# oritwoen/vgen

Hardware: AMD Instinct MI355X
Metric: Mkeys/sec (keys tried per second) (higher is better)
Workload: dtype u32

## Files before the change

vgen_amd/csrc/device/kernels.hip:

```cpp
#include <hip/hip_runtime.h>

#ifndef VG_PARK
#define VG_PARK 0
#endif
#ifndef VG_KECCAK_BLOCK
#define VG_KECCAK_BLOCK 1
#endif
#ifndef VG_PARKI
#define VG_PARKI 1
#endif
#define VG_HASH_BLOCKS 1
#include "../core/dfa_eval.h"
#include "../core/ec.h"
#include "../core/ed25519.h"
#include "../core/filter_eval.h"
#include "../core/hash.h"
#include "../core/rnd.h"
#include "../core/taproot.h"
#include "device_types.h"
#include "launch.h"

namespace vg {

constexpr int WG = SEQ_WG;

#ifndef VG_SEQ_WAVES_P2TR
#define VG_SEQ_WAVES_P2TR 2
#endif
#ifndef VG_SEQ_WAVES_ETH
#define VG_SEQ_WAVES_ETH 4
#endif


__device__ __forceinline__ void lds_store_fe(u32 *base, int stride, int col, const fe &a) {
#pragma unroll
    for (int i = 0; i < 9; i++) base[i * stride + col] = a.n[i];
}

__device__ __forceinline__ void lds_load_fe(const u32 *base, int stride, int col, fe &a) {
#pragma unroll
    for (int i = 0; i < 9; i++) a.n[i] = base[i * stride + col];
}

typedef __attribute__((address_space(3))) volatile u32 lds_vu32;

__device__ __forceinline__ void lds_park_fe(u32 *base, int stride, int col, const fe &a) {
    lds_vu32 *b = (lds_vu32 *)base;
#pragma unroll
    for (int i = 0; i < 9; i++) b[i * stride + col] = a.n[i];
}

__device__ __forceinline__ void lds_unpark_fe(u32 *base, int stride, int col, fe &a) {
    lds_vu32 *b = (lds_vu32 *)base;
#pragma unroll
    for (int i = 0; i < 9; i++) a.n[i] = b[i * stride + col];
}

__device__ __forceinline__ void fe_set_beta(fe &b) {
    b.n[0] = 0x119501EEu; b.n[1] = 0x09CB6143u; b.n[2] = 0x1D626570u; b.n[3] = 0x0092EA25u; b.n[4] = 0x034E99CFu;
    b.n[5] = 0x03CF561Au; b.n[6] = 0x1C41B991u; b.n[7] = 0x056CAF80u; b.n[8] = 0x007AE96Au;
}

__device__ __forceinline__ void shfl_xor_fe(fe &r, const fe &a, int mask) {
#pragma unroll
    for (int i = 0; i < 9; i++) r.n[i] = (u32)__shfl_xor((int)a.n[i], mask);
}

__device__ __forceinline__ u32 match_slot(DevMatchHeader *hdr, bool hit, u32 match_base) {
    const unsigned long long m = __ballot(hit);
    if (m == 0) return 0xFFFFFFFFu;
    const u32 rank = __builtin_amdgcn_mbcnt_hi((u32)(m >> 32), __builtin_amdgcn_mbcnt_lo((u32)m, 0u));
    const int leader = __ffsll((long long)m) - 1;
    u32 first = 0;
    if (hit && rank == 0) first = atomicAdd(&hdr->count, (u32)__popcll(m));
    first = (u32)__builtin_amdgcn_readlane((int)first, leader);
    return first + rank - match_base;
}

#include "hash_blocks.inc"


template <int FMT>
struct MatchFmt {
    static constexpr int value = (FMT == VGF_P2TR || vgf_is_eth(FMT)) ? -1 : FMT;
};

template <int FMT>
struct DumpOnly {
    static constexpr bool value = FMT == VGF_ETHEREUM_CONTRACT;
};

template <int FMT>
struct PayloadWords {
    static constexpr int value = (FMT == VGF_P2TR) ? 8 : 5;
};

template <int FMT, bool LONE = false>
__device__ __forceinline__ bool payload_from_point(const fe &x, const fe &y_canon, u32 *out) {
    static_assert(FMT != VGF_P2TR, "taproot payloads come from p2tr_tweak_kernel / p2tr_out_kernel");
    static_assert(!LONE || FMT == VGF_P2PKH, "the lone variant exists for the headline format only");
    u32 xw[8];
    fe_to_words(x, xw);
    if (LONE) {
        u32 sha[8];
        sha256_pub33(2u | (y_canon.n[0] & 1u), xw, sha);
        ripemd160_of_sha(sha, out);
    } else if (FMT == VGF_P2PKH || FMT == VGF_P2WPKH) {
        hash160_pub33_block(2u | (y_canon.n[0] & 1u), xw, out);
    } else if (FMT == VGF_P2SH_P2WPKH) {
        u32 h[5];
        hash160_pub33_block(2u | (y_canon.n[0] & 1u), xw, h);
        hash160_script22_block(h, out);
    } else if (FMT == VGF_P2PKH_UNCOMPRESSED) {
        u32 yw[8];
        fe_to_words(y_canon, yw);
        hash160_pub65_block(xw, yw, out);
    } else {
        u32 yw[8];
        fe_to_words(y_canon, yw);
#if VG_KECCAK_BLOCK
        keccak_addr_block(xw, yw, out);
#else
        keccak256_pub64_addr(xw, yw, out);
#endif
        if (FMT == VGF_ETHEREUM_CONTRACT) {
            u32 acc[5];
#pragma unroll
            for (int i = 0; i < 5; i++) acc[i] = out[i];
#if VG_KECCAK_BLOCK
            keccak_create_block(acc, out);
#else
            keccak256_create_addr(acc, out);
#endif
        }
    }
    return true;
}



__global__ void __launch_bounds__(WG) __attribute__((amdgpu_waves_per_eu(1, 8)))
seq_fwd_kernel(const SeqArgs args) {
    __builtin_amdgcn_s_setprio(3);
    __shared__ u32 tree[9 * WG];
    const int tid = threadIdx.x;
    const u32 S = args.s;
    const u32 lanes = args.lanes;
    const u32 u = blockIdx.x * WG + tid;

    fe rx;
#pragma unroll
    for (int i = 0; i < 9; i++) rx.n[i] = args.rtab[(size_t)i * lanes + u];

    u32 *pre = args.pre + u;
    fe acc;
#pragma unroll 1
    for (u32 j = 0; j < S; j++) {
        fe dx;
#pragma unroll
        for (int i = 0; i < 9; i++) dx.n[i] = rx.n[i] + args.q[j].nqx[i];
        if (j == 0) {
            acc = dx;
            fe_normalize_weak(acc);
        } else {
            fe_mul(acc, acc, dx);
        }
#pragma unroll
        for (int i = 0; i < 9; i++) pre[(size_t)(j * 9 + i) * lanes] = acc.n[i];
    }

    fe sib, pair;
    shfl_xor_fe(sib, acc, 1);
    fe_mul(pair, acc, sib);
    if ((tid & 1) == 0) lds_store_fe(tree, WG, WG / 2 + (tid >> 1), pair);
    __syncthreads();
    for (int width = WG / 4; width >= 1; width >>= 1) {
        if (tid < width) {
            const int k = width + tid;
            fe a, b, p;
            lds_load_fe(tree, WG, 2 * k, a);
            lds_load_fe(tree, WG, 2 * k + 1, b);
            fe_mul(p, a, b);
            lds_store_fe(tree, WG, k, p);
        }
        __syncthreads();
    }
    u32 *tg = args.tree + (size_t)blockIdx.x * 9 * WG;
#pragma unroll
    for (int i = 0; i < 9; i++) tg[i * WG + tid] = tree[i * WG + tid];
    if (tid < 9) args.root[(size_t)tid * args.groups + blockIdx.x] = tree[tid * WG + 1];
}


__global__ void __launch_bounds__(64) seq_inv_kernel(u32 *root, u32 groups) {
    __builtin_amdgcn_s_setprio(3);
    const u32 g = blockIdx.x * 64 + threadIdx.x;
    const u32 gg = g < groups ? g : groups - 1;
    fe r, ri;
#pragma unroll
    for (int i = 0; i < 9; i++) r.n[i] = root[(size_t)i * groups + gg];
    fe_inv(ri, r);
    if (g < groups) {
#pragma unroll
        for (int i = 0; i < 9; i++) root[(size_t)i * groups + g] = ri.n[i];
    }
}


__device__ __forceinline__ void tree_down_sweep(u32 *tree, int tid) {
    static_assert(WG % 64 == 0 && WG >= 128, "siblings c and c ^ 1 must be lanes of one 64-lane wave at every level");
    for (int width = 1; width <= WG / 4; width <<= 1) {
        if (tid < 2 * width) {
            const int c = 2 * width + tid;
            fe ik, sib, ic;
            lds_load_fe(tree, WG, c >> 1, ik);
            lds_load_fe(tree, WG, c ^ 1, sib);
            fe_mul(ic, ik, sib);
            __builtin_amdgcn_wave_barrier();
            lds_store_fe(tree, WG, c, ic);
        }
        __syncthreads();
    }
}

#ifndef VG_SEQ_WAVES_P2PKH
#define VG_SEQ_WAVES_P2PKH 4
#endif
#ifndef VG_SEQ_WAVES_P2SH
#define VG_SEQ_WAVES_P2SH 4
#endif
#ifndef VG_SEQ_WAVES_UNCOMP
#define VG_SEQ_WAVES_UNCOMP 4
#endif
#ifndef VG_SEQ_WAVES_FULL20
#define VG_SEQ_WAVES_FULL20 4
#endif
#ifndef VG_SEQ_WAVES_EC
#define VG_SEQ_WAVES_EC 4
#endif
#ifndef VG_SEQ_WAVES_HASH
#define VG_SEQ_WAVES_HASH 8
#endif
#ifndef VG_BASE_PRIO
#define VG_BASE_PRIO 1
#endif
#ifndef VG_EC_PRIO
#define VG_EC_PRIO 0
#endif
#ifndef VG_EC_SPRIO
#define VG_EC_SPRIO 0
#endif
#ifndef VG_SEQ_WAVES_HASH_FULL
#define VG_SEQ_WAVES_HASH_FULL 6
#endif
template <int FMT, bool FULL, bool ENDO = false>
struct SeqWaves {
    static constexpr int value = FMT == VGF_P2TR ? VG_SEQ_WAVES_P2TR : vgf_is_eth(FMT) ? (FULL && ENDO ? 3 : VG_SEQ_WAVES_ETH)
                                 : FULL ? VG_SEQ_WAVES_FULL20 : FMT == VGF_P2SH_P2WPKH ? VG_SEQ_WAVES_P2SH
                                 : FMT == VGF_P2PKH_UNCOMPRESSED ? VG_SEQ_WAVES_UNCOMP : VG_SEQ_WAVES_P2PKH;
};

template <int FMT, bool FULL, bool ENDO = false, bool LONE = false, bool SPLIT = false>
__global__ void __launch_bounds__(WG) __attribute__((amdgpu_waves_per_eu(SPLIT ? VG_SEQ_WAVES_EC : SeqWaves<FMT, FULL, ENDO>::value, SPLIT ? VG_SEQ_WAVES_EC : SeqWaves<FMT, FULL, ENDO>::value)))
seq_bwd_kernel(const SeqArgs args) {
#if VG_BASE_PRIO
    if (!SPLIT) __builtin_amdgcn_s_setprio(VG_BASE_PRIO);
#endif
#if VG_EC_PRIO
    if (SPLIT) __builtin_amdgcn_s_setprio(VG_EC_PRIO);
#endif
    static_assert(!SPLIT || (!FULL && !ENDO && !LONE && FMT == VGF_P2PKH), "the split form parks compressed keys: x and the parity of y");
    __shared__ u32 tree[9 * WG];
    __shared__ u32 ypark[ENDO && (FMT == VGF_P2PKH_UNCOMPRESSED || vgf_is_eth(FMT)) ? 9 * WG : 1];
    extern __shared__ u32 dyn_lds[];
    constexpr int NW = PayloadWords<FMT>::value;
    constexpr int PARKM = (!FULL && !ENDO && !LONE && (FMT == VGF_P2PKH || FMT == VGF_P2WPKH)) ? VG_PARK : 0;
    constexpr bool PARK = PARKM == 1, PARK2 = PARKM == 2;
    constexpr bool PARKI = VG_PARKI && !PARK && !PARK2 && !LONE && (FMT == VGF_P2PKH_UNCOMPRESSED || vgf_is_eth(FMT) || (FMT == VGF_P2PKH && FULL && ENDO));
    __shared__ u32 rpark[PARK ? 17 * WG : (PARK2 || PARKI) ? 9 * WG : 1];
    constexpr bool LEANMUL = !(FULL && ENDO) && (FMT == VGF_P2PKH || FMT == VGF_P2WPKH || FMT == VGF_P2SH_P2WPKH);
    const int tid = threadIdx.x;
    const GenTables gtab{args.gtab, args.gtab16, args.gtab_bits};
    u32 *dfa_lds = dyn_lds;
    if (FULL) {
        for (u32 i = tid; i < args.dfa_bytes / 4; i += WG) dfa_lds[i] = args.dfa_blob[i];
    }
    const u32 S = args.s;
    const u32 lanes = args.lanes;
    const u32 u = blockIdx.x * WG + tid;
    const bool stamp = FMT != VGF_P2TR && !SPLIT && blockIdx.x == 0 && args.mhdr != nullptr;
    const unsigned long long stamp_c0 = stamp ? clock64() : 0ull, stamp_w0 = stamp ? wall_clock64() : 0ull;

    const u32 *tg = args.tree + (size_t)blockIdx.x * 9 * WG;
#pragma unroll
    for (int i = 0; i < 9; i++) tree[i * WG + tid] = tg[i * WG + tid];
    __syncthreads();
    if (tid < 9) tree[tid * WG + 1] = args.root[(size_t)tid * args.groups + blockIdx.x];
    __syncthreads();
    tree_down_sweep(tree, tid);
    const u32 *pre = args.pre + u;
    fe inv;
    {
        fe ip, sib;
        lds_load_fe(tree, WG, WG / 2 + (tid >> 1), ip);
#pragma unroll
        for (int i = 0; i < 9; i++) sib.n[i] = args.pre[(size_t)((S - 1) * 9 + i) * lanes + (u ^ 1u)];
        fe_mul(inv, ip, sib);
    }
    if (ENDO || PARK || PARK2) __syncthreads();

    fe rx, ry;
    if (!PARK2) {
#pragma unroll
        for (int i = 0; i < 9; i++) {
            rx.n[i] = args.rtab[(size_t)i * lanes + u];
            ry.n[i] = args.rtab[(size_t)(9 + i) * lanes + u];
        }
    }
    if (PARK2) lds_park_fe(tree, WG, tid, inv);
    if (PARKI) lds_park_fe(rpark, WG, tid, inv);
    if (PARK) {
        lds_park_fe(rpark, WG, tid, rx);
        {
            lds_vu32 *b = (lds_vu32 *)(rpark + 9 * WG);
#pragma unroll
            for (int i = 0; i < 8; i++) b[i * WG + tid] = ry.n[i];
        }
        lds_park_fe(tree, WG, tid, inv);
    }

    const u32 half = args.n >> 1;
    const bool dump = DumpOnly<FMT>::value || args.dump != nullptr;
    fe zrun;
    u32 step = 0;

#pragma unroll 1
    for (int j = (int)S - 1; j >= 0; j--) {
        const DevSeqQ &q = args.q[j];
        fe dx, idx;
        if (PARK) {
            lds_unpark_fe(rpark, WG, tid, rx);
            lds_unpark_fe(tree, WG, tid, inv);
        }
        if (PARKI) lds_unpark_fe(rpark, WG, tid, inv);
        if (PARK2) {
            const u32 *rt = args.rtab + u;
            asm volatile("" : "+v"(rt));
#pragma unroll
            for (int i = 0; i < 9; i++) rx.n[i] = rt[(size_t)i * lanes];
            lds_unpark_fe(tree, WG, tid, inv);
        }
#pragma unroll
        for (int i = 0; i < 9; i++) dx.n[i] = rx.n[i] + q.nqx[i];
        if (j > 0) {
            fe pj;
#pragma unroll
            for (int i = 0; i < 9; i++) pj.n[i] = pre[(size_t)((j - 1) * 9 + i) * lanes];
            fe_mul(idx, inv, pj);
            fe_mul(inv, inv, dx);
            if (PARK || PARK2) lds_park_fe(tree, WG, tid, inv);
            if (PARKI) lds_park_fe(rpark, WG, tid, inv);
        } else {
            idx = inv;
        }
        if (PARK2) lds_park_fe(rpark, WG, tid, idx);
        if (!PARK && !PARK2) {
#pragma unroll
            for (int i = 0; i < 9; i++) {
                asm volatile("" : "+v"(rx.n[i]));
                asm volatile("" : "+v"(ry.n[i]));
            }
        }
        fe nsum, nqy;
        if (!PARK2) fe_neg(nsum, rx, 1);
#pragma unroll
        for (int i = 0; i < 9; i++) {
            if (!PARK2) nsum.n[i] += q.nqx[i];
            nqy.n[i] = q.nqy[i];
        }
#pragma unroll 1
        for (int sgn = 0; sgn < 2; sgn++) {
            fe dy, lam, x3, t, y3;
            if (PARK2) {
                const u32 *rt = args.rtab + u;
                asm volatile("" : "+v"(rt));
#pragma unroll
                for (int i = 0; i < 9; i++) {
                    rx.n[i] = rt[(size_t)i * lanes];
                    ry.n[i] = rt[(size_t)(9 + i) * lanes];
                }
                fe_neg(nsum, rx, 1);
#pragma unroll
                for (int i = 0; i < 9; i++) nsum.n[i] += q.nqx[i];
                lds_unpark_fe(rpark, WG, tid, idx);
            }
            if (PARK) {
                lds_vu32 *b = (lds_vu32 *)(rpark + 9 * WG);
#pragma unroll
                for (int i = 0; i < 8; i++) ry.n[i] = b[i * WG + tid];
            }
            if (sgn) fe_neg(dy, ry, 1);
            else dy = ry;
#pragma unroll
            for (int i = 0; i < 9; i++) dy.n[i] += q.nqy[i];
            fe_mul(lam, dy, idx);
            fe_sqr_add<LEANMUL>(x3, lam, nsum);
            if (VG_EC_SPRIO && !LONE) __builtin_amdgcn_s_setprio(0);
            fe_canonicalize_product(x3);
            fe_neg(t, x3, 1);
#pragma unroll
            for (int i = 0; i < 9; i++) t.n[i] += q.qx[i];
            if (VG_EC_SPRIO && !LONE) __builtin_amdgcn_s_setprio(VG_BASE_PRIO);
            fe_mul_add<LEANMUL>(y3, lam, t, nqy);
            if (VG_EC_SPRIO && !LONE) __builtin_amdgcn_s_setprio(0);
            if (FMT == VGF_P2PKH || FMT == VGF_P2WPKH || FMT == VGF_P2SH_P2WPKH)
                y3.n[0] = fe_parity_weak(y3);
            else
                fe_canonicalize_product(y3);

            if (FMT == VGF_P2TR) {
                gej qq;
                const bool okq = taproot_tweak_point(x3, y3, gtab, qq);
                const bool zero = taproot_z_is_zero(qq.z);
                if (zero) fe_set_one(qq.z);
                if (step == 0) zrun = qq.z;
                else fe_mul(zrun, zrun, qq.z);
                u32 *o = args.tq + (size_t)step * 27 * lanes + u;
#pragma unroll
                for (int i = 0; i < 9; i++) {
                    o[(size_t)i * lanes] = qq.x.n[i];
                    o[(size_t)(9 + i) * lanes] = qq.z.n[i];
                    o[(size_t)(18 + i) * lanes] = zrun.n[i];
                }
                args.tq_flag[(size_t)step * lanes + u] = (okq && !zero) ? 1u : 0u;
                step++;
                continue;
            }

            if (SPLIT) {
                u32 xw[8];
                fe_to_words(x3, xw);
                u32 *o = args.xs + (size_t)((u32)j * 2u + (u32)sgn) * lanes + u;
#pragma unroll
                for (int i = 0; i < 8; i++) o[(size_t)i * args.n] = xw[i];
                o[(size_t)8 * args.n] = 2u | (y3.n[0] & 1u);
                continue;
            }
            const u32 index = sgn ? (half - (u + 1) * S + (u32)j) : (half + u * S + (u32)j);
            if (ENDO) {
                constexpr bool NEEDS_Y = FMT == VGF_P2PKH_UNCOMPRESSED || vgf_is_eth(FMT);
                const u32 ypar = y3.n[0] & 1u;
                lds_park_fe(tree, WG, tid, x3);
                if (NEEDS_Y) lds_park_fe(ypark, WG, tid, y3);
#pragma unroll 1
                for (u32 v = 0; v < 6; v++) {
                    const u32 e = v >> 1, sneg = v & 1u;
                    fe xe, ye;
                    lds_unpark_fe(tree, WG, tid, xe);
                    if (sneg == 0 && e > 0) {
                        fe beta;
                        fe_set_beta(beta);
                        fe_mul(xe, xe, beta);
                        fe_canonicalize_product(xe);
                        lds_park_fe(tree, WG, tid, xe);
                    }
                    if (NEEDS_Y) {
                        lds_unpark_fe(ypark, WG, tid, ye);
                        if (sneg) {
                            fe ny;
                            fe_neg(ny, ye, 1);
                            fe_normalize(ny);
                            ye = ny;
                        }
                    } else {
                        ye.n[0] = ypar ^ sneg;
                    }
                    u32 ple[NW];
                    (void)payload_from_point<FMT == VGF_P2TR ? VGF_P2PKH : FMT>(xe, ye, ple);
                    const u32 vindex = (sneg * 3u + e) * args.n + index;
                    if (dump) {
                        u32 *o = args.dump + (size_t)vindex * NW;
#pragma unroll
                        for (int i = 0; i < NW; i++) o[i] = ple[i];
                    } else {
                        const bool hit = FULL ? dfa_match_payload_n<NW, MatchFmt<FMT>::value>(dfa_lds, (int)args.fmt, ple) : filter_eval_n<NW>(args.filter, ple);
                        const u32 slot = match_slot(args.mhdr, hit, args.match_base);
                        if (hit && slot < args.match_cap) {
                            DevMatch *m = args.mrec + slot;
                            m->index = vindex;
                            m->reserved = 0;
#pragma unroll
                            for (int i = 0; i < 8; i++) m->payload[i] = i < NW ? ple[i] : 0u;
                        }
                    }
                }
                continue;
            }

            u32 pl[NW];
            const bool ok = payload_from_point<FMT == VGF_P2TR ? VGF_P2PKH : FMT, LONE>(x3, y3, pl);

            if (dump) {
                u32 *o = args.dump + (size_t)index * NW;
#pragma unroll
                for (int i = 0; i < NW; i++) o[i] = ok ? pl[i] : 0u;
            } else {
                const bool hit = ok && (FULL ? dfa_match_payload_n<NW, MatchFmt<FMT>::value>(dfa_lds, (int)args.fmt, pl) : filter_eval_n<NW>(args.filter, pl));
                const u32 slot = match_slot(args.mhdr, hit, args.match_base);
                if (hit && slot < args.match_cap) {
                    DevMatch *m = args.mrec + slot;
                    m->index = index;
                    m->reserved = 0;
#pragma unroll
                    for (int i = 0; i < 8; i++) m->payload[i] = i < NW ? pl[i] : 0u;
                }
            }
        }
    }
    if (stamp && tid == 0) {
        args.mhdr->clk_cycles += (u32)(clock64() - stamp_c0);
        args.mhdr->clk_ticks += (u32)(wall_clock64() - stamp_w0);
    }
    if (FMT == VGF_P2TR) {
        __syncthreads();
        fe sib, pair;
        shfl_xor_fe(sib, zrun, 1);
        fe_mul(pair, zrun, sib);
        if ((tid & 1) == 0) lds_store_fe(tree, WG, WG / 2 + (tid >> 1), pair);
        __syncthreads();
#pragma unroll 1
        for (int width = WG / 4; width >= 1; width >>= 1) {
            if (tid < width) {
                const int k = width + tid;
                fe a, b, p;
                lds_load_fe(tree, WG, 2 * k, a);
                lds_load_fe(tree, WG, 2 * k + 1, b);
                fe_mul(p, a, b);
                lds_store_fe(tree, WG, k, p);
            }
            __syncthreads();
        }
        u32 *t2 = args.tree2 + (size_t)blockIdx.x * 9 * WG;
#pragma unroll
        for (int i = 0; i < 9; i++) t2[i * WG + tid] = tree[i * WG + tid];
        if (tid < 9) args.root2[(size_t)tid * args.groups + blockIdx.x] = tree[tid * WG + 1];
    }
}

template <int FMT, bool FULL>
struct HashWaves {
    static constexpr int value = FULL && FMT == VGF_P2PKH ? VG_SEQ_WAVES_HASH_FULL : VG_SEQ_WAVES_HASH;
};
template <int FMT, bool FULL>
__global__ void __launch_bounds__(WG) __attribute__((amdgpu_waves_per_eu(HashWaves<FMT, FULL>::value, HashWaves<FMT, FULL>::value)))
seq_hash_kernel(const SeqArgs args) {
#if VG_BASE_PRIO
    __builtin_amdgcn_s_setprio(VG_BASE_PRIO);
#endif
    static_assert(FMT == VGF_P2PKH || FMT == VGF_P2SH_P2WPKH, "compressed-key formats (P2WPKH shares P2PKH's payload)");
    extern __shared__ u32 dfa_lds[];
    const int tid = threadIdx.x;
    if (FULL) {
        for (u32 i = tid; i < args.dfa_bytes / 4; i += WG) dfa_lds[i] = args.dfa_blob[i];
        __syncthreads();
    }
    const u32 lanes = args.lanes, S = args.s, half = args.n >> 1;
    const u32 u = blockIdx.x * WG + tid;
    const bool stamp = blockIdx.x == 0 && blockIdx.y == 0 && args.mhdr != nullptr;
    const unsigned long long stamp_c0 = stamp ? clock64() : 0ull, stamp_w0 = stamp ? wall_clock64() : 0ull;
    const bool dump = args.dump != nullptr;
#pragma unroll 1
    for (u32 k = 0; k < args.hash_kpl; k++) {
        const u32 step = blockIdx.y * args.hash_kpl + k;
        const u32 *in = args.xs + (size_t)step * lanes + u;
        u32 xw[8];
#pragma unroll
        for (int i = 0; i < 8; i++) xw[i] = in[(size_t)i * args.n];
        const u32 prefix = in[(size_t)8 * args.n];
        u32 pl[5];
        if (FMT == VGF_P2SH_P2WPKH) {
            u32 h[5];
            hash160_pub33_block(prefix, xw, h);
            hash160_script22_block(h, pl);
        } else {
            hash160_pub33_block(prefix, xw, pl);
        }
        const u32 j = step >> 1, sgn = step & 1u;
        const u32 index = sgn ? (half - (u + 1) * S + j) : (half + u * S + j);
        if (dump) {
            u32 *o = args.dump + (size_t)index * 5;
#pragma unroll
            for (int i = 0; i < 5; i++) o[i] = pl[i];
        } else {
            const bool hit = FULL ? dfa_match_payload_n<5, MatchFmt<FMT>::value>(dfa_lds, (int)args.fmt, pl) : filter_eval_n<5>(args.filter, pl);
            const u32 slot = match_slot(args.mhdr, hit, args.match_base);
            if (hit && slot < args.match_cap) {
                DevMatch *m = args.mrec + slot;
                m->index = index;
                m->reserved = 0;
#pragma unroll
                for (int i = 0; i < 8; i++) m->payload[i] = i < 5 ? pl[i] : 0u;
            }
        }
    }
    if (stamp && tid == 0) {
        args.mhdr->clk_cycles += (u32)(clock64() - stamp_c0);
        args.mhdr->clk_ticks += (u32)(wall_clock64() - stamp_w0);
    }
}

#ifndef VG_XONLY_WAVES
#define VG_XONLY_WAVES 5
#endif
#ifndef VG_XONLY_WAVES_MATCH
#define VG_XONLY_WAVES_MATCH 4
#endif
template <bool PRE, bool ENDO>
struct XonlyWaves {
    static constexpr int value = (PRE || ENDO) ? VG_XONLY_WAVES_MATCH : VG_XONLY_WAVES;
};

__device__ __forceinline__ void xonly_store_hits(unsigned long long *hits, u32 bits, u32 u, u32 S, u32 half, u32 image_base) {
    const u32 G = 64u / S, l = u & (G - 1u), field = (1u << S) - 1u;
    unsigned long long wp = (unsigned long long)(bits & field) << (l * S);
    unsigned long long wn = (unsigned long long)((bits >> 16) & field) << ((G - 1u - l) * S);
    for (u32 m = 1; m < G; m <<= 1) {
        wp |= ((unsigned long long)(u32)__shfl_xor((int)(wp >> 32), (int)m) << 32) | (u32)__shfl_xor((int)wp, (int)m);
        wn |= ((unsigned long long)(u32)__shfl_xor((int)(wn >> 32), (int)m) << 32) | (u32)__shfl_xor((int)wn, (int)m);
    }
    if (l == 0) {
        hits[(image_base + half + u * S) >> 6] = wp;
        hits[(image_base + half - (u + G) * S) >> 6] = wn;
    }
}

__device__ __forceinline__ void xonly_payload(const fe &x, u32 out[8]) {
    u32 xw[8];
    fe_to_words(x, xw);
#pragma unroll
    for (int i = 0; i < 8; i++) out[i] = bswap32(xw[7 - i]);
}

template <bool PRE, bool ENDO>
__global__ void __launch_bounds__(WG) __attribute__((amdgpu_waves_per_eu(XonlyWaves<PRE, ENDO>::value, XonlyWaves<PRE, ENDO>::value)))
xonly_bwd_kernel(const SeqArgs args) {
    __shared__ u32 tree[9 * WG];
    const int tid = threadIdx.x;
    const u32 S = args.s;
    const u32 lanes = args.lanes;
    const u32 u = blockIdx.x * WG + tid;

    const u32 *tg = args.tree + (size_t)blockIdx.x * 9 * WG;
#pragma unroll
    for (int i = 0; i < 9; i++) tree[i * WG + tid] = tg[i * WG + tid];
    __syncthreads();
    if (tid < 9) tree[tid * WG + 1] = args.root[(size_t)tid * args.groups + blockIdx.x];
    __syncthreads();
    for (int width = 1; width <= WG / 4; width <<= 1) {
        if (tid < width) {
            const int k = width + tid;
            fe ik, a, b, ia, ib;
            lds_load_fe(tree, WG, k, ik);
            lds_load_fe(tree, WG, 2 * k, a);
            lds_load_fe(tree, WG, 2 * k + 1, b);
            fe_mul(ia, ik, b);
            fe_mul(ib, ik, a);
            lds_store_fe(tree, WG, 2 * k, ia);
            lds_store_fe(tree, WG, 2 * k + 1, ib);
        }
        __syncthreads();
    }
    const u32 *pre = args.pre + u;
    fe inv;
    {
        fe ip, sib;
        lds_load_fe(tree, WG, WG / 2 + (tid >> 1), ip);
#pragma unroll
        for (int i = 0; i < 9; i++) sib.n[i] = args.pre[(size_t)((S - 1) * 9 + i) * lanes + (u ^ 1u)];
        fe_mul(inv, ip, sib);
    }
    fe rx, ry;
#pragma unroll
    for (int i = 0; i < 9; i++) {
        rx.n[i] = args.rtab[(size_t)i * lanes + u];
        ry.n[i] = args.rtab[(size_t)(9 + i) * lanes + u];
    }
    const u32 half = args.n >> 1;
    u32 hbits0 = 0, hbits1 = 0, hbits2 = 0;

#pragma unroll 1
    for (int j = (int)S - 1; j >= 0; j--) {
        const DevSeqQ &q = args.q[j];
        fe dx, idx;
#pragma unroll
        for (int i = 0; i < 9; i++) dx.n[i] = rx.n[i] + q.nqx[i];
        if (j > 0) {
            fe pj;
#pragma unroll
            for (int i = 0; i < 9; i++) pj.n[i] = pre[(size_t)((j - 1) * 9 + i) * lanes];
            fe_mul(idx, inv, pj);
            fe_mul(inv, inv, dx);
        } else {
            idx = inv;
        }
#pragma unroll
        for (int i = 0; i < 9; i++) {
            asm volatile("" : "+v"(rx.n[i]));
            asm volatile("" : "+v"(ry.n[i]));
        }
        fe nsum;
        fe_neg(nsum, rx, 1);
#pragma unroll
        for (int i = 0; i < 9; i++) nsum.n[i] += q.nqx[i];
#pragma unroll 1
        for (int sgn = 0; sgn < 2; sgn++) {
            fe dy, lam, x3;
            if (sgn) fe_neg(dy, ry, 1);
            else dy = ry;
#pragma unroll
            for (int i = 0; i < 9; i++) dy.n[i] += q.nqy[i];
            fe_mul(lam, dy, idx);
            fe_sqr_add(x3, lam, nsum);
            fe_canonicalize_product(x3);
            const u32 index = sgn ? (half - (u + 1) * S + (u32)j) : (half + u * S + (u32)j);
#pragma unroll 1
            for (u32 e = 0; e < (ENDO ? 3u : 1u); e++) {
                if (ENDO && e > 0) {
                    fe beta;
                    fe_set_beta(beta);
                    fe_mul(x3, x3, beta);
                    fe_canonicalize_product(x3);
                }
                u32 pl[8];
                xonly_payload(x3, pl);
                const u32 vindex = ENDO ? e * args.n + index : index;
                u32 *o = args.dump + (size_t)vindex * 8;
                if (!PRE) {
#pragma unroll
                    for (int i = 0; i < 8; i++) o[i] = pl[i];
                } else {
                    const bool hit = filter_eval_npub(args.filter, pl);
                    const u32 bit = (hit ? 1u : 0u) << ((u32)j + (sgn ? 16u : 0u));
                    hbits0 |= e == 0 ? bit : 0u;
                    if (ENDO) {
                        hbits1 |= e == 1 ? bit : 0u;
                        hbits2 |= e == 2 ? bit : 0u;
                    }
                    if (hit) {
#pragma unroll
                        for (int i = 0; i < 8; i++) o[i] = pl[i];
                    }
// ... 1697 lines not shown
```

Measured before the change: 16410.

## Enable register-parking mode that reloads rx/ry from global and raises occupancy

```diff
diff --git a/vgen_amd/csrc/device/kernels.hip b/vgen_amd/csrc/device/kernels.hip
--- a/vgen_amd/csrc/device/kernels.hip
+++ b/vgen_amd/csrc/device/kernels.hip
@@ -1,7 +1,7 @@
 #include <hip/hip_runtime.h>
 
 #ifndef VG_PARK
-#define VG_PARK 0
+#define VG_PARK 1
 #endif
 #ifndef VG_KECCAK_BLOCK
 #define VG_KECCAK_BLOCK 1
@@ -43,6 +43,12 @@
 }
 
 typedef __attribute__((address_space(3))) volatile u32 lds_vu32;
+
+__device__ __forceinline__ u32 load_row_word(const u32 *table, u32 lanes, int row, u32 off) {
+    unsigned long long r = (unsigned long long)(table + (size_t)row * lanes);
+    asm("" : "+s"(r));
+    return *(const __attribute__((address_space(1))) u32 *)(r + off);
+}
 
 __device__ __forceinline__ void lds_park_fe(u32 *base, int stride, int col, const fe &a) {
     lds_vu32 *b = (lds_vu32 *)base;
@@ -253,15 +259,23 @@
 #ifndef VG_SEQ_WAVES_HASH_FULL
 #define VG_SEQ_WAVES_HASH_FULL 6
 #endif
-template <int FMT, bool FULL, bool ENDO = false>
+#ifndef VG_SEQ_WAVES_PARK
+#define VG_SEQ_WAVES_PARK 6
+#endif
+template <int FMT, bool FULL, bool ENDO, bool LONE, bool SPLIT>
+struct SeqPark {
+    static constexpr bool value = VG_PARK && !FULL && !ENDO && !LONE && !SPLIT && (FMT == VGF_P2PKH || FMT == VGF_P2WPKH);
+};
+template <int FMT, bool FULL, bool ENDO = false, bool LONE = false, bool SPLIT = false>
 struct SeqWaves {
-    static constexpr int value = FMT == VGF_P2TR ? VG_SEQ_WAVES_P2TR : vgf_is_eth(FMT) ? (FULL && ENDO ? 3 : VG_SEQ_WAVES_ETH)
+    static constexpr int value = SPLIT ? VG_SEQ_WAVES_EC : SeqPark<FMT, FULL, ENDO, LONE, SPLIT>::value ? VG_SEQ_WAVES_PARK
+                                 : FMT == VGF_P2TR ? VG_SEQ_WAVES_P2TR : vgf_is_eth(FMT) ? (FULL && ENDO ? 3 : VG_SEQ_WAVES_ETH)
                                  : FULL ? VG_SEQ_WAVES_FULL20 : FMT == VGF_P2SH_P2WPKH ? VG_SEQ_WAVES_P2SH
                                  : FMT == VGF_P2PKH_UNCOMPRESSED ? VG_SEQ_WAVES_UNCOMP : VG_SEQ_WAVES_P2PKH;
 };
 
 template <int FMT, bool FULL, bool ENDO = false, bool LONE = false, bool SPLIT = false>
-__global__ void __launch_bounds__(WG) __attribute__((amdgpu_waves_per_eu(SPLIT ? VG_SEQ_WAVES_EC : SeqWaves<FMT, FULL, ENDO>::value, SPLIT ? VG_SEQ_WAVES_EC : SeqWaves<FMT, FULL, ENDO>::value)))
+__global__ void __launch_bounds__(WG) __attribute__((amdgpu_waves_per_eu(SeqWaves<FMT, FULL, ENDO, LONE, SPLIT>::value, SeqWaves<FMT, FULL, ENDO, LONE, SPLIT>::value)))
 seq_bwd_kernel(const SeqArgs args) {
 #if VG_BASE_PRIO
     if (!SPLIT) __builtin_amdgcn_s_setprio(VG_BASE_PRIO);
@@ -274,10 +288,9 @@
     __shared__ u32 ypark[ENDO && (FMT == VGF_P2PKH_UNCOMPRESSED || vgf_is_eth(FMT)) ? 9 * WG : 1];
     extern __shared__ u32 dyn_lds[];
     constexpr int NW = PayloadWords<FMT>::value;
-    constexpr int PARKM = (!FULL && !ENDO && !LONE && (FMT == VGF_P2PKH || FMT == VGF_P2WPKH)) ? VG_PARK : 0;
-    constexpr bool PARK = PARKM == 1, PARK2 = PARKM == 2;
-    constexpr bool PARKI = VG_PARKI && !PARK && !PARK2 && !LONE && (FMT == VGF_P2PKH_UNCOMPRESSED || vgf_is_eth(FMT) || (FMT == VGF_P2PKH && FULL && ENDO));
-    __shared__ u32 rpark[PARK ? 17 * WG : (PARK2 || PARKI) ? 9 * WG : 1];
+    constexpr bool PARK = SeqPark<FMT, FULL, ENDO, LONE, SPLIT>::value;
+    constexpr bool PARKI = VG_PARKI && !PARK && !LONE && (FMT == VGF_P2PKH_UNCOMPRESSED || vgf_is_eth(FMT) || (FMT == VGF_P2PKH && FULL && ENDO));
+    __shared__ u32 rpark[PARKI ? 9 * WG : 1];
     constexpr bool LEANMUL = !(FULL && ENDO) && (FMT == VGF_P2PKH || FMT == VGF_P2WPKH || FMT == VGF_P2SH_P2WPKH);
     const int tid = threadIdx.x;
     const GenTables gtab{args.gtab, args.gtab16, args.gtab_bits};
@@ -307,30 +320,23 @@
         for (int i = 0; i < 9; i++) sib.n[i] = args.pre[(size_t)((S - 1) * 9 + i) * lanes + (u ^ 1u)];
         fe_mul(inv, ip, sib);
     }
-    if (ENDO || PARK || PARK2) __syncthreads();
+    if (ENDO || PARK) __syncthreads();
 
     fe rx, ry;
-    if (!PARK2) {
+    if (!PARK) {
 #pragma unroll
         for (int i = 0; i < 9; i++) {
             rx.n[i] = args.rtab[(size_t)i * lanes + u];
             ry.n[i] = args.rtab[(size_t)(9 + i) * lanes + u];
         }
     }
-    if (PARK2) lds_park_fe(tree, WG, tid, inv);
+    if (PARK) lds_park_fe(tree, WG, tid, inv);
     if (PARKI) lds_park_fe(rpark, WG, tid, inv);
-    if (PARK) {
-        lds_park_fe(rpark, WG, tid, rx);
-        {
-            lds_vu32 *b = (lds_vu32 *)(rpark + 9 * WG);
-#pragma unroll
-            for (int i = 0; i < 8; i++) b[i * WG + tid] = ry.n[i];
-        }
-        lds_park_fe(tree, WG, tid, inv);
-    }
 
     const u32 half = args.n >> 1;
     const bool dump = DumpOnly<FMT>::value || args.dump != nullptr;
+    u32 ipos = half + u * S;
+    if (PARK) asm volatile("" : "+v"(ipos));
     fe zrun;
     u32 step = 0;
 
@@ -338,16 +344,12 @@
     for (int j = (int)S - 1; j >= 0; j--) {
         const DevSeqQ &q = args.q[j];
         fe dx, idx;
+        if (PARKI) lds_unpark_fe(rpark, WG, tid, inv);
         if (PARK) {
-            lds_unpark_fe(rpark, WG, tid, rx);
-            lds_unpark_fe(tree, WG, tid, inv);
-        }
-        if (PARKI) lds_unpark_fe(rpark, WG, tid, inv);
-        if (PARK2) {
-            const u32 *rt = args.rtab + u;
-            asm volatile("" : "+v"(rt));
-#pragma unroll
-            for (int i = 0; i < 9; i++) rx.n[i] = rt[(size_t)i * lanes];
+            u32 ro = u * 4u;
+            asm volatile("" : "+v"(ro));
+#pragma unroll
+            for (int i = 0; i < 9; i++) rx.n[i] = load_row_word(args.rtab, lanes, i, ro);
             lds_unpark_fe(tree, WG, tid, inv);
         }
 #pragma unroll
@@ -358,13 +360,12 @@
             for (int i = 0; i < 9; i++) pj.n[i] = pre[(size_t)((j - 1) * 9 + i) * lanes];
             fe_mul(idx, inv, pj);
             fe_mul(inv, inv, dx);
-            if (PARK || PARK2) lds_park_fe(tree, WG, tid, inv);
+            if (PARK) lds_park_fe(tree, WG, tid, inv);
             if (PARKI) lds_park_fe(rpark, WG, tid, inv);
         } else {
             idx = inv;
         }
-        if (PARK2) lds_park_fe(rpark, WG, tid, idx);
-        if (!PARK && !PARK2) {
+        if (!PARK) {
 #pragma unroll
             for (int i = 0; i < 9; i++) {
                 asm volatile("" : "+v"(rx.n[i]));
@@ -372,32 +373,26 @@
             }
         }
         fe nsum, nqy;
-        if (!PARK2) fe_neg(nsum, rx, 1);
+        if (!PARK) fe_neg(nsum, rx, 1);
 #pragma unroll
         for (int i = 0; i < 9; i++) {
-            if (!PARK2) nsum.n[i] += q.nqx[i];
+            if (!PARK) nsum.n[i] += q.nqx[i];
             nqy.n[i] = q.nqy[i];
         }
 #pragma unroll 1
         for (int sgn = 0; sgn < 2; sgn++) {
             fe dy, lam, x3, t, y3;
-            if (PARK2) {
-                const u32 *rt = args.rtab + u;
-                asm volatile("" : "+v"(rt));
+            if (PARK) {
+                u32 ro = u * 4u;
+                asm volatile("" : "+v"(ro));
 #pragma unroll
                 for (int i = 0; i < 9; i++) {
-                    rx.n[i] = rt[(size_t)i * lanes];
-                    ry.n[i] = rt[(size_t)(9 + i) * lanes];
+                    rx.n[i] = load_row_word(args.rtab, lanes, i, ro);
+                    ry.n[i] = load_row_word(args.rtab, lanes, i, ro + 36u * lanes);
                 }
                 fe_neg(nsum, rx, 1);
 #pragma unroll
                 for (int i = 0; i < 9; i++) nsum.n[i] += q.nqx[i];
-                lds_unpark_fe(rpark, WG, tid, idx);
-            }
-            if (PARK) {
-                lds_vu32 *b = (lds_vu32 *)(rpark + 9 * WG);
-#pragma unroll
-                for (int i = 0; i < 8; i++) ry.n[i] = b[i * WG + tid];
             }
             if (sgn) fe_neg(dy, ry, 1);
             else dy = ry;
@@ -446,7 +441,8 @@
                 o[(size_t)8 * args.n] = 2u | (y3.n[0] & 1u);
                 continue;
             }
-            const u32 index = sgn ? (half - (u + 1) * S + (u32)j) : (half + u * S + (u32)j);
+            const u32 index = PARK ? (sgn ? (2u * half - S + (u32)j) - ipos : ipos + (u32)j)
+                                   : sgn ? (half - (u + 1) * S + (u32)j) : (half + u * S + (u32)j);
             if (ENDO) {
                 constexpr bool NEEDS_Y = FMT == VGF_P2PKH_UNCOMPRESSED || vgf_is_eth(FMT);
                 const u32 ypar = y3.n[0] & 1u;
```

Result: no change. 16510 (median of 6 runs) (+0.6%).
